# jinilover/floydWarshall

Measured on AMD Instinct MI355X. Metric: edge-relaxations/sec (N^3/t), N=16384 fp32, higher is better.
Workload: dtype f32

## Files before the change

floydwarshall_amd/_lib.py:

```python
import ctypes
import os

os.environ.setdefault("HSA_ENABLE_IPC_MODE_LEGACY", "0")

PKG = os.path.dirname(os.path.abspath(__file__))
LIB_PATH = os.environ.get("FWX_LIB_PATH") or os.path.join(PKG, "libfwx.so")

FWX_OK = 0
FWX_ERR_INVALID = -1
FWX_ERR_NO_DEVICE = -2
FWX_ERR_HIP = -3
FWX_ERR_OOM = -4
FWX_ERR_CYCLE = -5
FWX_ERR_CAPACITY = -6
FWX_ERR_UNSUPPORTED = -7
FWX_ERR_RCCL = -8
FWX_ERR_INTERNAL = -9

FWX_ABI_VERSION = 3
FWX_F32, FWX_F64 = 0, 1
FWX_ENGINE_AUTO, FWX_ENGINE_PERK, FWX_ENGINE_FUSED = 0, 1, 2
FWX_UPDATE_SHARDS = 256
FWX_FUSED_BLOCK = 64
FWX_BATCH_MAX_N = 128
# ... 42 lines not shown

class FwxMultiTiming(ctypes.Structure):
    _fields_ = [("struct_size", ctypes.c_uint32), ("steps", c_i32), ("pivots_per_step", c_i32),
                ("partitions", c_i32), ("bulk_us", ctypes.c_float), ("bulk_mean_us", ctypes.c_float),
                ("lookahead_us", ctypes.c_float), ("panel_us", ctypes.c_float),
                ("exchange_us", ctypes.c_float), ("chain_us", ctypes.c_float),
                ("chain_over_bulk", ctypes.c_float)]


class FwxError(RuntimeError):
    def __init__(self, status, what):
        self.status = status
        msg = lib().fwx_strerror(status).decode()
        extra = ""
        if status == FWX_ERR_HIP:
            extra = " (hipError_t %d)" % lib().fwx_last_hip_error()
        super().__init__("%s: %s%s" % (what, msg, extra))


SIGNATURES = {
    "fwx_abi_version": (ctypes.c_int, []),
    "fwx_device_count": (ctypes.c_int, []),
    "fwx_strerror": (ctypes.c_char_p, [ctypes.c_int]),
    "fwx_last_hip_error": (ctypes.c_int, []),
    "fwx_hip_versions": (ctypes.c_int, [ctypes.POINTER(c_i32), ctypes.POINTER(c_i32)]),
    "fwx_test_fail_after": (ctypes.c_int, [c_i32]),
    "fwx_test_kernel_forms": (ctypes.c_int, [ctypes.POINTER(ctypes.c_uint64), ctypes.c_int]),
    "fwx_test_kernel_form_name": (ctypes.c_char_p, [ctypes.c_int]),
    "fwx_test_perk_pivots": (ctypes.c_int, [ctypes.POINTER(ctypes.c_uint64), ctypes.c_int]),
    "fwx_test_perk_fold": (ctypes.c_int, []),
    "fwx_test_perk_walk": (ctypes.c_int, []),
    "fwx_test_perk_deep": (ctypes.c_int, [ctypes.POINTER(ctypes.c_uint64), ctypes.c_int]),
    "fwx_test_perk_tile": (ctypes.c_int, [ctypes.POINTER(ctypes.c_uint64), ctypes.c_int]),
    "fwx_test_perk_wide": (ctypes.c_int, [ctypes.POINTER(ctypes.c_uint64), ctypes.c_int]),
    "fwx_solve_f64": (ctypes.c_int, [c_i32, c_vp, c_vp, c_vp, ctypes.POINTER(FwxOpts)]),
    "fwx_solve_f32": (ctypes.c_int, [c_i32, c_vp, c_vp, c_vp, ctypes.POINTER(FwxOpts)]),
    "fwx_follow_path": (ctypes.c_int, [c_i32, c_vp, c_i32, c_i32, c_vp, c_i32]),
    "fwx_matrix_create": (ctypes.c_int, [ctypes.POINTER(c_vp), c_i32, c_i32, c_i32, c_i32, c_i32]),
    "fwx_matrix_upload": (ctypes.c_int, [c_vp, c_vp, c_vp, c_vp]),
    "fwx_matrix_solve": (ctypes.c_int, [c_vp, ctypes.POINTER(FwxOpts)]),
    "fwx_matrix_download": (ctypes.c_int, [c_vp, c_vp, c_vp, c_vp]),
    "fwx_matrix_query": (ctypes.c_int, [c_vp, c_i32, c_i32, ctypes.POINTER(ctypes.c_double), c_vp,
                                        c_i32]),
    "fwx_matrix_destroy": (ctypes.c_int, [c_vp]),
    "fwx_matrix_keep_input": (ctypes.c_int, [c_vp]),
    "fwx_matrix_patch_input": (ctypes.c_int, [c_vp, c_i32, c_vp, c_vp, c_vp, c_vp]),
    "fwx_matrix_enable_resume": (ctypes.c_int, [c_vp, c_i32]),
    "fwx_matrix_resume_bytes": (ctypes.c_int, [c_vp, c_i32, ctypes.POINTER(ctypes.c_uint64)]),
    "fwx_device_memory": (ctypes.c_int, [c_i32, ctypes.POINTER(ctypes.c_uint64),
                                         ctypes.POINTER(ctypes.c_uint64)]),
    "fwx_matrix_resolve": (ctypes.c_int, [c_vp, c_i32, c_vp, c_vp, c_vp, c_vp, ctypes.POINTER(FwxOpts),
                                          ctypes.POINTER(c_i32)]),
    "fwx_matrix_enable_path_log": (ctypes.c_int, [c_vp]),
    "fwx_matrix_path_log_count": (ctypes.c_int, [c_vp, ctypes.POINTER(ctypes.c_uint64)]),
    "fwx_matrix_query_exact": (ctypes.c_int, [c_vp, c_i32, c_i32, ctypes.POINTER(ctypes.c_double),
                                              c_vp, c_i32]),
    "fwx_matrix_query_exact_batch": (ctypes.c_int, [c_vp, c_i32, c_vp, c_vp, c_vp, c_vp, c_i32]),
    "fwx_matrix_create_multi": (ctypes.c_int, [ctypes.POINTER(c_vp), c_i32, c_i32, c_i32, c_i32, c_i32,
                                               ctypes.POINTER(c_i32), c_i32]),
    "fwx_matrix_create_part": (ctypes.c_int, [ctypes.POINTER(c_vp), c_i32, c_i32, c_i32, c_i32, c_i32, c_i32, c_i32,
                                              c_vp, c_vp]),
    "fwx_matrix_part_rows": (ctypes.c_int, [c_vp, c_i32, ctypes.POINTER(c_i32), ctypes.POINTER(c_i32)]),
    "fwx_matrix_domain_bits": (ctypes.c_int, [c_vp, ctypes.POINTER(c_i32)]),
    "fwx_matrix_set_domain": (ctypes.c_int, [c_vp, c_i32]),
    "fwx_matrix_parts": (ctypes.c_int, [c_vp, ctypes.POINTER(c_i32)]),
    "fwx_matrix_set_timing": (ctypes.c_int, [c_vp, c_i32]),
# ... 106 lines not shown
```

floydwarshall_amd/csrc/fwx_api.hip:

```cpp
#include <hip/hip_runtime.h>
#include <stddef.h>
#include <stdint.h>
#include <stdlib.h>
#include <string.h>

#include <cmath>
#include <new>

#include "fwx.h"
#include "fwx_guard.h"
#include "fwx_handle.h"
#include "fwx_internal.h"
#include "fwx_kernels.h"
#include "fwx_query.h"

using namespace fwxi;

namespace {

template <typename T>
int fused_block(const fwx_slab *sl, int k0, int bt, const T *w, const int32_t *wh,
                const fwx_fused_scratch *sc, const fwx_trace *tr, unsigned long long *d_updates,
                bool nonneg, hipStream_t s, int skip_lo = 0, int skip_hi = 0)
{
// ... 821 lines not shown
    return fwx::KF_COUNT;
}

int fwx_test_perk_pivots(uint64_t *launches, int reset)
{
    for (int i = 0; i < 5; ++i) {
        const uint64_t v = reset ? g_perk_launches[i].exchange(0, std::memory_order_relaxed)
                                 : g_perk_launches[i].load(std::memory_order_relaxed);
        if (launches) launches[i] = v;
    }
    return perk_pivots();
}

int fwx_test_perk_fold(void) { return perk_fold_compare() ? 1 : 0; }

int fwx_test_perk_walk(void) { return perk_walk() ? 1 : 0; }

int fwx_test_perk_deep(uint64_t *deep_launches, int reset)
{
    const uint64_t v = reset ? g_perk_deep_launches.exchange(0, std::memory_order_relaxed)
                             : g_perk_deep_launches.load(std::memory_order_relaxed);
    if (deep_launches) *deep_launches = v;
    return perk_deep() ? 1 : 0;
}

int fwx_test_perk_tile(uint64_t *launches, int reset)
{
    const uint64_t v = reset ? g_perk_tile_launches.exchange(0, std::memory_order_relaxed)
                             : g_perk_tile_launches.load(std::memory_order_relaxed);
    if (launches) *launches = v;
    return perk_tile_min_n();
}

int fwx_test_perk_wide(uint64_t *wide_launches, int reset)
{
    const uint64_t v = reset ? g_perk_wide_launches.exchange(0, std::memory_order_relaxed)
                             : g_perk_wide_launches.load(std::memory_order_relaxed);
    if (wide_launches) *wide_launches = v;
    return perk_wide() ? 1 : 0;
}

const char *fwx_test_kernel_form_name(int form)
{
    static const char *const names[] = {
#define FWX_KERNEL_FORM_NAME(name) #name,
        FWX_KERNEL_FORM_LIST(FWX_KERNEL_FORM_NAME)
#undef FWX_KERNEL_FORM_NAME
    };
    return form >= 0 && form < fwx::KF_COUNT ? names[form] : nullptr;
}

const char *fwx_strerror(int status)
{
    switch (status) {
    case FWX_OK: return "ok";
    case FWX_ERR_INVALID: return "invalid argument";
    case FWX_ERR_NO_DEVICE: return "no HIP device visible (libfwx has no CPU fallback)";
    case FWX_ERR_HIP: return "HIP runtime error";
    case FWX_ERR_OOM: return "out of memory";
    case FWX_ERR_CYCLE: return "next-hop walk does not reach the destination (cycle)";
    case FWX_ERR_CAPACITY: return "output buffer too small";
    case FWX_ERR_UNSUPPORTED: return "unsupported option combination";
    case FWX_ERR_RCCL: return "RCCL could not be loaded or an RCCL call failed";
    case FWX_ERR_INTERNAL: return "internal error (an exception was stopped at the C ABI)";
    default: return "unknown status";
    }
// ... 691 lines not shown
```

floydwarshall_amd/csrc/fwx_fused.hip:

```cpp
#include <hip/hip_runtime.h>
#include <type_traits>
#include <stdint.h>
#include <stdlib.h>

#include "fwx_kernels.h"

#pragma clang fp contract(off)

namespace fwx {

namespace {

template <typename T> __device__ __forceinline__ T qnan();
template <> __device__ __forceinline__ float qnan<float>() { return __builtin_nanf(""); }
template <> __device__ __forceinline__ double qnan<double>() { return __builtin_nan(""); }

__device__ __forceinline__ float fmax_t(float a, float b)
{
    float d;
    asm("v_max_f32 %0, %1, %2" : "=v"(d) : "v"(a), "v"(b));
    return d;
}
__device__ __forceinline__ double fmax_t(double a, double b)
{
// ... 946 lines not shown
        for (int q = 0; q < RI / 4; ++q) {
            const F32x4 cv = *reinterpret_cast<const F32x4 *>(&sCp[u][ti * RI + q * 4]);
#pragma unroll
            for (int e = 0; e < 4; ++e) c[q * 4 + e] = cv[e];
        }
#pragma unroll
        for (int h = 0; h < NH; ++h) {
            const F32x4 wq = *reinterpret_cast<const F32x4 *>(&sWp[u][h * 64 + tj * 4]);
#pragma unroll
            for (int e = 0; e < 4; ++e) wv[h][e] = wq[e];
        }
#pragma unroll
        for (int r = 0; r < RI; ++r)
#pragma unroll
            for (int h = 0; h < NH; ++h)
#pragma unroll
                for (int e = 0; e < 4; ++e) {
                    float p;
                    asm("v_mul_f32 %0, %1, %2" : "=v"(p) : "v"(c[r]), "v"(wv[h][e]));
                    x[r][h][e] = x[r][h][e] < p ? p : x[r][h][e];
                }
    }
}

__device__ __forceinline__ int sign_bits(F32x4 v)
{
    typedef int I4 __attribute__((ext_vector_type(4)));
    const I4 b = __builtin_bit_cast(I4, v);
    return b[0] | b[1] | b[2] | b[3];
}

template <int MINW, int RI, int NH>
__global__ __launch_bounds__(256, MINW) void relax_tile(float *rate, int n, int k0, const float *w,
                                                        const float *ct, int ct_ld, int force_cmp)
{
    typedef float V4 __attribute__((ext_vector_type(4)));
    constexpr int TI = 16 * RI, TJ = 64 * NH, HJ = 64, BS = 16, HP = BS / 2, NS = B / BS;
    static_assert(TI == 128 && TJ == 128, "every thread stages both operands: 8 pivot pairs x 32 vectors");

    __shared__ __attribute__((aligned(16))) float sW[2][HP][2][TJ];
    __shared__ __attribute__((aligned(16))) float sC[2][HP][2][TI];
    __shared__ __attribute__((aligned(16))) int sVote[2][4];

    const int tid = threadIdx.x;
    const int i_base = blockIdx.y * TI;
    const int j_base = blockIdx.x * TJ;
    const int ti = tid >> 4, tj = tid & 15;
    const int i0 = i_base + ti * RI;
    const int sp = tid >> 5, sv = tid & 31;

    auto voted = [&](int buf) -> bool {
        typedef int I4 __attribute__((ext_vector_type(4)));
        const I4 v = *reinterpret_cast<const I4 *>(&sVote[buf][0]);
        return __builtin_amdgcn_readfirstlane(v[0] | v[1] | v[2] | v[3]) != 0;
    };
    auto x_bits = [&](const V4 (&x)[RI][NH]) -> int {
        unsigned m = 0;
#pragma unroll
        for (int r = 0; r < RI; ++r)
#pragma unroll
            for (int h = 0; h < NH; ++h)
#pragma unroll
                for (int e = 0; e < 4; ++e) {
                    const float f = x[r][h][e];
                    const unsigned b = __builtin_bit_cast(unsigned, f);
                    m = b > m ? b : m;
                }
        return m > 0x7f800000u ? (int)0x80000000u : 0;
    };
    const bool interior = i_base + TI <= n && j_base + TJ <= n &&
                          !(i_base < j_base + TJ && j_base < i_base + TI) &&
                          (k0 + B <= j_base || k0 >= j_base + TJ);

    const float nanv = qnan<float>();
    const int sj = j_base + sv * 4, si = i_base + sv * 4;
    const bool sj_ok = sj < n, si_ok = si < n;
    const float *wp = w + (size_t)(2 * sp) * n + (sj_ok ? sj : 0);
    const float *cp = ct + (size_t)(2 * sp) * ct_ld + (si_ok ? si : 0);
    int kcol = k0 + 2 * sp - sj;
    V4 pw[2], pc[2];
    auto prefetch = [&]() {
        pw[0] = *reinterpret_cast<const V4 *>(wp);
        pw[1] = *reinterpret_cast<const V4 *>(wp + n);
        pc[0] = *reinterpret_cast<const V4 *>(cp);
        pc[1] = *reinterpret_cast<const V4 *>(cp + ct_ld);
        wp += (size_t)BS * n;
        cp += (size_t)BS * ct_ld;
    };
    auto commit = [&](int buf, int extra) {
        int bits = extra;
#pragma unroll
        for (int u = 0; u < 2; ++u) {
            V4 a = pw[u], c = pc[u];
#pragma unroll
            for (int e = 0; e < 4; ++e) {
                a[e] = (!sj_ok || kcol + u == e) ? nanv : a[e];
                c[e] = si_ok ? c[e] : nanv;
            }
            *reinterpret_cast<V4 *>(&sW[buf][sp][u][sv * 4]) = a;
            *reinterpret_cast<V4 *>(&sC[buf][sp][u][sv * 4]) = c;
            bits |= sign_bits(a) | sign_bits(c);
        }
        kcol += BS;
        sVote[buf][tid >> 6] = __builtin_amdgcn_ballot_w64(bits < 0) != 0 ? 1 : 0;
    };

    prefetch();
    V4 x[RI][NH];
    if (interior) {
        const float *xp = rate + (size_t)i0 * n + j_base + tj * 4;
#pragma unroll
        for (int r = 0; r < RI; ++r)
#pragma unroll
            for (int h = 0; h < NH; ++h) x[r][h] = *reinterpret_cast<const V4 *>(xp + (size_t)r * n + h * HJ);
    } else {
#pragma unroll
        for (int r = 0; r < RI; ++r) {
            const int i = min(i0 + r, n - 1);
#pragma unroll
            for (int h = 0; h < NH; ++h) {
                const int j = j_base + h * HJ + tj * 4;
                x[r][h] = *reinterpret_cast<const V4 *>(rate + (size_t)i * n + (j < n ? j : n - 4));
            }
        }
    }
    __builtin_amdgcn_s_waitcnt(FWX_WAIT_VMCNT0);
    commit(0, x_bits(x));
    __syncthreads();

    bool cmp = force_cmp != 0;
    int buf = 0;
#pragma unroll 1
    for (int s = 0; s < NS; ++s, buf ^= 1) {
        const bool more = s + 1 < NS;
        cmp |= voted(buf);
        if (more) prefetch();
        const int nmax = cmp ? 0 : HP;
#pragma unroll 1
        for (int tp = 0; tp < nmax; ++tp) max_fold_pair<RI, NH>(sW[buf][tp], sC[buf][tp], ti, tj, x);
#pragma unroll 1
        for (int tp = nmax; tp < HP; ++tp) cmp_fold_pair<RI, NH>(sW[buf][tp], sC[buf][tp], ti, tj, x);
        if (more) {
            commit(buf ^ 1, 0);
            __syncthreads();
        }
    }

    if (interior) {
        float *xp = rate + (size_t)i0 * n + j_base + tj * 4;
#pragma unroll
        for (int r = 0; r < RI; ++r)
#pragma unroll
            for (int h = 0; h < NH; ++h) *reinterpret_cast<V4 *>(xp + (size_t)r * n + h * HJ) = x[r][h];
        return;
    }
    if (i_base < j_base + TJ && j_base < i_base + TI) {
#pragma unroll
        for (int r = 0; r < RI; ++r) {
            const int i = i0 + r;
            if (i >= n) continue;
#pragma unroll
            for (int h = 0; h < NH; ++h) {
                const int j = j_base + h * HJ + tj * 4;
                if (i >= j && i < j + 4) x[r][h][i - j] = rate[(size_t)i * n + i];
            }
        }
        __builtin_amdgcn_s_waitcnt(FWX_WAIT_VMCNT0);
// ... 1276 lines not shown
            return hipGetLastError();
        }
        if (tight && a.next && !a.hops) {
            note_form(a.plog.last ? KF_PANELS_NEXT_TRACE_F32 : KF_PANELS_NEXT_F32);
            if (a.plog.last)
                hipLaunchKernelGGL(fused_panels_next_f32<true>, grid, block, 0, s, row_wgs, a.rate, a.next, a.n, a.k0,
                                   a.bt, w_out, a.ct, a.cnt, a.ct_ld, a.plog.last, a.plog.at_row, a.plog.at_col);
            else
                hipLaunchKernelGGL(fused_panels_next_f32<false>, grid, block, 0, s, row_wgs, a.rate, a.next, a.n, a.k0,
                                   a.bt, w_out, a.ct, a.cnt, a.ct_ld, nullptr, nullptr, nullptr);
            return hipGetLastError();
        }
    }
    const bool max_form = !a.plog.last && !a.next && a.nonneg;
    note_form(sizeof(T) == 4 ? (max_form ? KF_PANELS_MAX_F32 : KF_PANELS_F32)
                             : (max_form ? KF_PANELS_MAX_F64 : KF_PANELS_F64));
    if (a.plog.last) {
        if (a.hops) FWX_PANELS(true, true, true); else FWX_PANELS(true, true, false);
    } else if (a.next) {
        if (a.hops) FWX_PANELS(true, false, true); else FWX_PANELS(true, false, false);
    } else if (a.nonneg) {
        hipLaunchKernelGGL((fused_panels<T, false, false, false, true>), grid, block, 0, s, row_wgs, a.rate,
                           a.next, a.n, a.k0, a.bt, w_out, a.ct, a.cnt, a.ct_ld, a.plog.last, a.plog.at_row,
                           a.plog.at_col, a.hops, wh_out, a.cht);
    } else {
        FWX_PANELS(false, false, false);
    }
#undef FWX_PANELS
    return hipGetLastError();
}
template hipError_t launch_fused_panels<float>(const FusedArgs<float> &, float *, int32_t *, hipStream_t);
template hipError_t launch_fused_panels<double>(const FusedArgs<double> &, double *, int32_t *, hipStream_t);

hipError_t launch_relax_tile(const RelaxKtArgs<float> &a, hipStream_t s)
{
    if (a.n <= 0) return hipSuccess;
    if (a.np != B || a.n < B || a.n % 4 || a.ct_ld % 4 || a.ct_ld < a.n || (uintptr_t)a.rate % 16 || (uintptr_t)a.w % 16 ||
        (uintptr_t)a.ct % 16 || a.k < 0 || a.k + a.np > a.n || a.updates)
        return hipErrorInvalidValue;
    const unsigned tiles = (unsigned)((a.n + 127) / 128);
    note_form(KF_RELAX_K);
    hipLaunchKernelGGL((relax_tile<3, 8, 2>), dim3(tiles, tiles), dim3(256), 0, s, a.rate, a.n, a.k, a.w, a.ct,
                       a.ct_ld, a.fold_compare ? 1 : 0);
    return hipGetLastError();
}

template hipError_t launch_fused_relax<float>(const FusedArgs<float> &, hipStream_t, int, int);
template hipError_t launch_fused_relax<double>(const FusedArgs<double> &, hipStream_t, int, int);
template hipError_t launch_fused_colpanel<float>(const FusedArgs<float> &, hipStream_t);
template hipError_t launch_fused_colpanel<double>(const FusedArgs<double> &, hipStream_t);
template hipError_t launch_fused_main<float>(const FusedArgs<float> &, int, int, hipStream_t, int,
                                             int, FusedCols);
template hipError_t launch_fused_main<double>(const FusedArgs<double> &, int, int, hipStream_t, int,
                                              int, FusedCols);
template hipError_t launch_fused_panel<float>(const float *, int, int, int, float *, hipStream_t, PathLog,
                                              const int32_t *, int32_t *);
template hipError_t launch_fused_panel<double>(const double *, int, int, int, double *, hipStream_t,
                                               PathLog, const int32_t *, int32_t *);

}

#ifdef FWX_CLOCK_PROBE
extern "C" __attribute__((visibility("default"))) int fwx_debug_clock(unsigned long long *out, int reset)
{
    if (out && hipMemcpyFromSymbol(out, HIP_SYMBOL(fwx::g_clk), 24) != hipSuccess) return -1;
    if (reset) {
        const unsigned long long z[3] = {0, 0, 0};
        if (hipMemcpyToSymbol(HIP_SYMBOL(fwx::g_clk), z, 24) != hipSuccess) return -1;
    }
    return 0;
}
#endif
```

floydwarshall_amd/csrc/fwx_internal.h:

```cpp
#ifndef FWX_INTERNAL_H
#define FWX_INTERNAL_H

#include <hip/hip_runtime.h>
#include <algorithm>
#include <mutex>
#include <new>
#include <type_traits>
#include <vector>
#include <limits.h>
#include <stddef.h>
#include <stdlib.h>
#include <stdint.h>
#include <string.h>

#include "fwx.h"
#include "fwx_kernels.h"

static_assert(FWX_UPDATE_SHARDS == FWX_UPDATE_SHARDS_K, "shard count mismatch");

namespace fwxi {

inline thread_local int g_last_hip = 0;

#define FWX_HIP(call)                                                                              \
// ... 383 lines not shown

#define FWX_PERK_PIVOTS_DEFAULT 8
inline int perk_pivots()
{
    if (const char *e = getenv("FWX_PERK_PIVOTS")) {
        char *end = nullptr;
        const long v = strtol(e, &end, 10);
        if (end != e && *end == '\0' && (v == 1 || v == 2 || v == 4 || v == 8)) return (int)v;
    }
    return FWX_PERK_PIVOTS_DEFAULT;
}

inline bool perk_wide()
{
    const char *e = getenv("FWX_PERK_WIDE");
    return !(e && !strcmp(e, "0"));
}

inline bool perk_walk()
{
    const char *e = getenv("FWX_PERK_WALK");
    return !(e && !strcmp(e, "0"));
}

inline bool perk_deep()
{
    const char *e = getenv("FWX_PERK_DEEP");
    return !(e && !strcmp(e, "0"));
}

#define FWX_PERK_TILE_MIN_N_DEFAULT 1024
inline int perk_tile_min_n() { return (int)env_digits("FWX_PERK_TILE_MIN_N", 0, INT_MAX, FWX_PERK_TILE_MIN_N_DEFAULT); }

inline bool perk_fold_compare()
{
    const char *e = getenv("FWX_PERK_FOLD");
    return e && !strcmp(e, "compare");
}

#define FWX_BATCH_WAVE_MAX_N_DEFAULT FWX_BATCH_WAVE_N
inline int batch_wave_max_n()
{
    return (int)env_digits("FWX_BATCH_WAVE_MAX_N", 0, FWX_BATCH_WAVE_N, FWX_BATCH_WAVE_MAX_N_DEFAULT);
}

#define FWX_BATCH_MID_MIN_N_DEFAULT (FWX_BATCH_MAX_N + 1)
inline int batch_mid_min_n()
{
    return (int)env_digits("FWX_BATCH_MID_MIN_N", 1, FWX_BATCH_MID_MIN_N_DEFAULT, FWX_BATCH_MID_MIN_N_DEFAULT);
}

#define FWX_BATCH_LARGE_MIN_N_DEFAULT (FWX_BATCH_MID_MAX_N + 1)
inline int batch_large_min_n()
{
    return (int)env_digits("FWX_BATCH_LARGE_MIN_N", 1, FWX_BATCH_LARGE_MIN_N_DEFAULT, FWX_BATCH_LARGE_MIN_N_DEFAULT);
}

#define FWX_BATCH_LISTS_BUDGET_BYTES ((long long)64 << 20)
inline long long batch_lists_chunk(int n, int cap)
{
    const long long per_item = 4ll * ((long long)cap + 3ll * ((long long)n + 2) + 4);
    long long fit = FWX_BATCH_LISTS_BUDGET_BYTES / per_item;
    if (fit < 1) fit = 1;
    return env_digits("FWX_BATCH_LISTS_CHUNK", 1, fit - 1, fit);
}

inline std::atomic<uint64_t> g_perk_launches[5];
inline std::atomic<uint64_t> g_perk_wide_launches;
inline std::atomic<uint64_t> g_perk_deep_launches;
inline std::atomic<uint64_t> g_perk_tile_launches;

template <typename T> inline size_t perk_kt_ws_bytes(int n)
{
    const size_t ld = ((size_t)n + 3) & ~(size_t)3;
    return (size_t)FWX_FUSED_B * ((size_t)n + ld) * sizeof(T);
}
class PerkScratch {
public:
    static int get(hipStream_t s, size_t bytes, void **out)
    {
        int dev = 0, cur = 0;
        FWX_HIP(hipGetDevice(&cur));
        dev = cur;
        if (s) FWX_HIP(hipStreamGetDevice(s, &dev));
        Pool &p = pool();
        std::lock_guard<std::mutex> lk(p.mu);
        Entry *e = nullptr;
        for (Entry &x : p.all)
            if (x.s == s && x.dev == dev) { e = &x; break; }
        if (!e) {
            if (p.all.size() >= kMax) {
                size_t lru = 0;
                for (size_t i = 1; i < p.all.size(); ++i)
                    if (p.all[i].used < p.all[lru].used) lru = i;
                if (p.all[lru].p) (void)hipFree(p.all[lru].p);
                p.all.erase(p.all.begin() + (long)lru);
            }
            p.all.push_back(Entry{dev, s, nullptr, 0, 0});
            e = &p.all.back();
        }
        e->used = ++p.clock;
        if (e->cap < bytes) {
            if (e->p) {
                if (s) (void)hipStreamSynchronize(s);
                (void)hipFree(e->p);
                e->p = nullptr; e->cap = 0;
            }
            if (dev != cur) FWX_HIP(hipSetDevice(dev));
            const hipError_t err = hipMalloc(&e->p, bytes);
            if (dev != cur) (void)hipSetDevice(cur);
            FWX_HIP(err);
            e->cap = bytes;
        }
        *out = e->p;
        return FWX_OK;
    }

private:
    static constexpr size_t kMax = 16;
    struct Entry { int dev; hipStream_t s; void *p; size_t cap; uint64_t used; };
    struct Pool { std::mutex mu; std::vector<Entry> all; uint64_t clock = 0; };
    static Pool &pool() { static Pool *p = new Pool(); return *p; }
};

template <typename T>
inline int relax_range_kt(T *rate, int n, int k_begin, int k_end, int serpentine, int np,
                          unsigned long long *d_updates, hipStream_t s, void *ws)
{
    const size_t ld = ((size_t)n + 3) & ~(size_t)3;
    if (!ws) {
        const int rc0 = PerkScratch::get(s, perk_kt_ws_bytes<T>(n), &ws);
        if (rc0) return rc0;
    }
    T *const w = (T *)ws, *const ct = w + (size_t)FWX_FUSED_B * n;

    fwx::FusedArgs<T> pa;
    pa.rate = rate; pa.next = nullptr; pa.rows = n; pa.n = n; pa.row0 = 0; pa.w = nullptr; pa.ct = ct;
    pa.cnt = nullptr; pa.ct_ld = (int)ld; pa.updates = nullptr; pa.nonneg = false;
    fwx::RelaxKtArgs<T> a;
    a.rate = rate; a.ct_ld = (int)ld; a.n = n; a.updates = d_updates;
    a.temporal_bytes = perk_temporal_bytes((size_t)n * n * sizeof(T));
    a.store_bytes = perk_store_bytes();
    a.fold_compare = perk_fold_compare();
    a.walk = perk_walk();
    fwx::RelaxArgs<T> a1;
    a1.rate = rate; a1.next = nullptr; a1.hops = nullptr; a1.phops = nullptr; a1.rows = n; a1.n = n; a1.row0 = 0;
    a1.updates = d_updates; a1.temporal_bytes = a.temporal_bytes; a1.store_bytes = a.store_bytes;
    const int rev = FWX_XCD_SERPENTINE && a.temporal_bytes >= 0 ? 2 : 1;
    Throttle thr;
    int sweeps = 0;
    auto after = [&](hipError_t e, int slot, int groups = 1) -> int {
        if (e == hipErrorInvalidValue) return FWX_ERR_INVALID;
        FWX_HIP(e);
        g_perk_launches[slot].fetch_add((uint64_t)groups, std::memory_order_relaxed);
        if (groups >= 2) g_perk_wide_launches.fetch_add((uint64_t)groups / 2, std::memory_order_relaxed);
        if (groups >= 4) g_perk_deep_launches.fetch_add((uint64_t)groups / 4, std::memory_order_relaxed);
        if (groups == 8) g_perk_tile_launches.fetch_add(1, std::memory_order_relaxed);
        return thr.tick(s);
    };
    const bool wide = np == 8 && !d_updates && std::is_same<T, float>::value && perk_wide();
    const int g_top = wide ? (a.walk && perk_deep() ? 32 : 16) : np;
    const int tile_min_n = perk_tile_min_n();
    const bool tile = g_top == 32 && tile_min_n > 0 && n >= tile_min_n && n >= FWX_FUSED_B;
    for (int k0 = k_begin; k0 < k_end; k0 += FWX_FUSED_B) {
        const int bt = std::min(FWX_FUSED_B, k_end - k0);
        int t = 0;
        if (bt >= 2) {
            pa.k0 = k0; pa.bt = bt;
            if (const int rc = after(fwx::launch_fused_panels<T>(pa, w, nullptr, s), 4)) return rc;
            if constexpr (std::is_same<T, float>::value) {
                if (tile && bt == FWX_FUSED_B) {
                    a.k = k0; a.np = bt; a.w = w; a.ct = ct;
                    a.flip = 0;
                    if (const int rc = after(fwx::launch_relax_tile(a, s), 3, 8)) return rc;
                    t = bt;
                }
            }
            for (int g = g_top; g >= 2; g >>= 1)
                for (; bt - t >= g; t += g) {
                    a.k = k0 + t; a.np = g; a.w = w + (size_t)t * n; a.ct = ct + (size_t)t * ld;
                    a.flip = serpentine ? rev * (sweeps++ & 1) : 0;
                    if (const int rc = after(fwx::launch_relax_kt<T>(a, s), g >= 8 ? 3 : g == 4 ? 2 : 1, g >= 16 ? g / 8 : 1))
                        return rc;
                }
        }
        for (; t < bt; ++t) {
            a1.k = k0 + t; a1.prow = rate + (size_t)a1.k * n;
            a1.flip = serpentine ? rev * (sweeps++ & 1) : 0;
            if (const int rc = after(fwx::launch_relax<T>(a1, s), 0)) return rc;
        }
    }
    return FWX_OK;
}

template <typename T>
inline int relax_range(T *rate, int32_t *next, int32_t *hops, int rows, int n, int row0, const T *prow0,
                const int32_t *phops0, int64_t stride, int k_begin, int k_end, int serpentine,
                unsigned long long *d_updates, hipStream_t s, fwx::PathLog plog = fwx::PathLog(),
                int skip_lo = 0, int skip_hi = 0, const int32_t *pnext0 = nullptr, void *kt_ws = nullptr)
{
    const int np = perk_pivots();
    if (np > 1 && !next && !hops && !plog.last && row0 == 0 && rows == n && skip_hi <= skip_lo &&
        n % (16 / (int)sizeof(T)) == 0 && (uintptr_t)rate % 16 == 0 && stride == n &&
        prow0 == rate + (size_t)k_begin * n && k_end - k_begin >= 2)
        return relax_range_kt<T>(rate, n, k_begin, k_end, serpentine, np, d_updates, s, kt_ws);
    fwx::RelaxArgs<T> a;
    Throttle thr;
    a.rate = rate; a.next = next; a.hops = hops;
    a.rows = rows; a.n = n; a.row0 = row0; a.updates = d_updates; a.plog = plog;
    a.skip_lo = skip_lo; a.skip_hi = skip_hi;
    a.temporal_bytes = perk_temporal_bytes((size_t)rows * n * sizeof(T));
    a.store_bytes = perk_store_bytes();
    const int rev = FWX_XCD_SERPENTINE && a.temporal_bytes >= 0 ? 2 : 1;
    for (int k = k_begin; k < k_end; ++k) {
        a.prow = prow0 + (int64_t)(k - k_begin) * stride;
        a.phops = phops0 ? phops0 + (int64_t)(k - k_begin) * stride : nullptr;
        a.pnext = pnext0 ? pnext0 + (int64_t)(k - k_begin) * stride : nullptr;
        a.k = k;
        a.flip = serpentine ? rev * (k & 1) : 0;
        const hipError_t e = fwx::launch_relax<T>(a, s);
        if (e == hipErrorInvalidValue) return FWX_ERR_INVALID;
        FWX_HIP(e);
        const int rc = thr.tick(s);
        if (rc) return rc;
    }
// ... 27 lines not shown
```

floydwarshall_amd/csrc/fwx_kernels.h:

```cpp
#ifndef FWX_KERNELS_H
#define FWX_KERNELS_H

#include <hip/hip_runtime.h>
#include <stdint.h>

#include <atomic>

#define FWX_UPDATE_SHARDS_K 256

namespace fwx {

struct PathLog {
    int32_t *last = nullptr;
    int32_t *at_col = nullptr;
    int32_t *at_row = nullptr;
};

#define FWX_KERNEL_FORM_LIST(X)                                                                    \
    X(SMALL_SOLVE)                                              \
    X(RELAX_K)                                                      \
    X(ROWPANEL_F32)                                                        \
    X(ROWPANEL_F64)                                                                                \
    X(COLPANEL_F32)                                                     \
    X(COLPANEL_F64)                                                                                \
// ... 46 lines not shown
    int flip;
    long long temporal_bytes = -1;
    int store_bytes = 0;
    int skip_lo = 0, skip_hi = 0;
    unsigned long long *updates;
    PathLog plog;
};

template <typename T> hipError_t launch_relax(const RelaxArgs<T> &a, hipStream_t s);

#define FWX_PERK_KT_RPB 8
#define FWX_PERK_KT_UNROLL 8
#define FWX_PERK_KT16_RPB 16
#define FWX_PERK_KT16_UNROLL 8
#define FWX_PERK_WALK_RPB 16
#define FWX_PERK_WALK_UNROLL 8
#define FWX_PERK_WALK_POL 0
#define FWX_PERK_WALK_ROLL false
#define FWX_PERK_DEEP_RPB 64
#define FWX_PERK_DEEP_UNROLL 8
template <typename T> struct RelaxKtArgs {
    T *rate;
    const T *w;
    const T *ct;
    int ct_ld, n, k, np;
    int flip;
    long long temporal_bytes = -1;
    int store_bytes = 0;
    bool fold_compare = false;
    bool walk = false;
    unsigned long long *updates = nullptr;
};
template <typename T> hipError_t launch_relax_kt(const RelaxKtArgs<T> &a, hipStream_t s);
hipError_t launch_relax_tile(const RelaxKtArgs<float> &a, hipStream_t s);

#define FWX_SMALL_N 128
template <typename T>
hipError_t launch_small_solve(T *rate, int32_t *next, int32_t *hops, int n, int k_begin, int k_end,
                              unsigned long long *updates, PathLog plog, hipStream_t s);

#define FWX_BATCH_WAVE_N 16
template <typename T>
hipError_t launch_batch_solve(T *rate, int32_t *next, int32_t *hops, int count, int n, long long stride,
                              int k_begin, int k_end, unsigned long long *updates_each, int wave_max_n,
                              hipStream_t s, PathLog plog = PathLog());

#define FWX_MID_N 256
#ifndef FWX_MID_B
#define FWX_MID_B 16
#endif
template <typename T>
hipError_t launch_batch_mid(T *rate, int32_t *next, int32_t *hops, int count, int n, long long stride, int k_begin,
                            int k_end, unsigned long long *updates_each, hipStream_t s, PathLog plog = PathLog());

#define FWX_LARGE_N 1024
#define FWX_LARGE_B 16
#define FWX_LARGE_S 48
#ifndef FWX_LARGE_TR
#define FWX_LARGE_TR 16
#endif
#ifndef FWX_LARGE_ROWS
#define FWX_LARGE_ROWS 4
#endif
#ifndef FWX_LARGE_TC
#define FWX_LARGE_TC 256
#endif
#define FWX_LARGE_SCRATCH_BYTES(n) ((size_t)(n) * (2 * FWX_LARGE_B * 16))
// ... 69 lines not shown
```

include/fwx.h:

```cpp
#ifndef FWX_H
#define FWX_H

#include <stddef.h>
#include <stdint.h>

#ifdef __cplusplus
extern "C" {
#endif

#define FWX_ABI_VERSION 3

typedef enum fwx_status {
    FWX_OK = 0,
    FWX_ERR_INVALID = -1,
    FWX_ERR_NO_DEVICE = -2,
    FWX_ERR_HIP = -3,
    FWX_ERR_OOM = -4,
    FWX_ERR_CYCLE = -5,
    FWX_ERR_CAPACITY = -6,
    FWX_ERR_UNSUPPORTED = -7,
    FWX_ERR_RCCL = -8,
    FWX_ERR_INTERNAL = -9
} fwx_status;

// ... 3 lines not shown
    FWX_ENGINE_AUTO = 0,
    FWX_ENGINE_PERK = 1,
    FWX_ENGINE_FUSED = 2
} fwx_engine;

typedef struct fwx_opts {
    uint32_t struct_size;
    int32_t device;
    int32_t engine;
    int32_t k_begin;
    int32_t k_end;
    int32_t block;
    int32_t serpentine;
    uint64_t *updates_out;
    void *stream;
    int32_t use_stream;
    int32_t reserved0;
} fwx_opts;

int fwx_abi_version(void);
int fwx_device_count(void);
const char *fwx_strerror(int status);
int fwx_last_hip_error(void);
int fwx_hip_versions(int32_t *built_against, int32_t *runtime);
int fwx_test_fail_after(int32_t countdown);
int fwx_test_kernel_forms(uint64_t *seen, int reset);
const char *fwx_test_kernel_form_name(int form);
int fwx_test_perk_pivots(uint64_t *launches, int reset);
int fwx_test_perk_wide(uint64_t *wide_launches, int reset);
int fwx_test_perk_fold(void);
int fwx_test_perk_walk(void);
int fwx_test_perk_deep(uint64_t *deep_launches, int reset);
int fwx_test_perk_tile(uint64_t *launches, int reset);

int fwx_solve_f64(int32_t n, double *rate, int32_t *next, int32_t *hops, const fwx_opts *opts);
int fwx_solve_f32(int32_t n, float *rate, int32_t *next, int32_t *hops, const fwx_opts *opts);

#define FWX_BATCH_MAX_N 128
int fwx_solve_batch_f64(int32_t count, int32_t n, double *rate, int32_t *next, int32_t *hops,
                        uint64_t *updates_each, const fwx_opts *opts);
int fwx_solve_batch_f32(int32_t count, int32_t n, float *rate, int32_t *next, int32_t *hops,
                        uint64_t *updates_each, const fwx_opts *opts);
int fwx_dev_solve_batch(int32_t count, int32_t n, int32_t dtype, void *rate, int32_t *next, int32_t *hops,
                        int64_t stride, int32_t k_begin, int32_t k_end,
                        unsigned long long *d_updates_each, void *stream);
int fwx_test_batch_wave_max_n(void);

#define FWX_BATCH_MID_MAX_N 256
int fwx_solve_batch_mid_f64(int32_t count, int32_t n, double *rate, int32_t *next, int32_t *hops,
                            uint64_t *updates_each, const fwx_opts *opts);
int fwx_solve_batch_mid_f32(int32_t count, int32_t n, float *rate, int32_t *next, int32_t *hops,
                            uint64_t *updates_each, const fwx_opts *opts);
int fwx_dev_solve_batch_mid(int32_t count, int32_t n, int32_t dtype, void *rate, int32_t *next, int32_t *hops,
                            int64_t stride, int32_t k_begin, int32_t k_end,
                            unsigned long long *d_updates_each, void *stream);
int fwx_test_batch_mid_min_n(void);
int fwx_test_batch_mid_block(void);

#define FWX_BATCH_LARGE_MAX_N 1024
#define FWX_BATCH_LARGE_SCRATCH_BYTES(n) ((size_t)(n) * 512)
int fwx_solve_batch_large_f64(int32_t count, int32_t n, double *rate, int32_t *next, int32_t *hops,
                              uint64_t *updates_each, const fwx_opts *opts);
int fwx_solve_batch_large_f32(int32_t count, int32_t n, float *rate, int32_t *next, int32_t *hops,
                              uint64_t *updates_each, const fwx_opts *opts);
int fwx_dev_solve_batch_large(int32_t count, int32_t n, int32_t dtype, void *rate, int32_t *next, int32_t *hops,
                              int64_t stride, int32_t k_begin, int32_t k_end,
// ... 229 lines not shown
```

Baseline: 28220 billion.

## Pair pivot blocks in tile relax and overlap next panels on side stream

```diff
diff --git a/floydwarshall_amd/_lib.py b/floydwarshall_amd/_lib.py
--- a/floydwarshall_amd/_lib.py
+++ b/floydwarshall_amd/_lib.py
@@ -98,6 +98,7 @@
     "fwx_test_perk_walk": (ctypes.c_int, []),
     "fwx_test_perk_deep": (ctypes.c_int, [ctypes.POINTER(ctypes.c_uint64), ctypes.c_int]),
     "fwx_test_perk_tile": (ctypes.c_int, [ctypes.POINTER(ctypes.c_uint64), ctypes.c_int]),
+    "fwx_test_perk_pair": (ctypes.c_int, [ctypes.POINTER(ctypes.c_uint64), ctypes.c_int]),
     "fwx_test_perk_wide": (ctypes.c_int, [ctypes.POINTER(ctypes.c_uint64), ctypes.c_int]),
     "fwx_solve_f64": (ctypes.c_int, [c_i32, c_vp, c_vp, c_vp, ctypes.POINTER(FwxOpts)]),
     "fwx_solve_f32": (ctypes.c_int, [c_i32, c_vp, c_vp, c_vp, ctypes.POINTER(FwxOpts)]),
diff --git a/floydwarshall_amd/csrc/fwx_api.hip b/floydwarshall_amd/csrc/fwx_api.hip
--- a/floydwarshall_amd/csrc/fwx_api.hip
+++ b/floydwarshall_amd/csrc/fwx_api.hip
@@ -877,6 +877,14 @@
     return perk_tile_min_n();
 }
 
+int fwx_test_perk_pair(uint64_t *launches, int reset)
+{
+    const uint64_t v = reset ? g_perk_pair_launches.exchange(0, std::memory_order_relaxed)
+                             : g_perk_pair_launches.load(std::memory_order_relaxed);
+    if (launches) *launches = v;
+    return perk_pair_min_n();
+}
+
 int fwx_test_perk_wide(uint64_t *wide_launches, int reset)
 {
     const uint64_t v = reset ? g_perk_wide_launches.exchange(0, std::memory_order_relaxed)
diff --git a/floydwarshall_amd/csrc/fwx_fused.hip b/floydwarshall_amd/csrc/fwx_fused.hip
--- a/floydwarshall_amd/csrc/fwx_fused.hip
+++ b/floydwarshall_amd/csrc/fwx_fused.hip
@@ -1002,19 +1002,35 @@
 
 template <int MINW, int RI, int NH>
 __global__ __launch_bounds__(256, MINW) void relax_tile(float *rate, int n, int k0, const float *w,
-                                                        const float *ct, int ct_ld, int force_cmp)
+                                                        const float *ct, int ct_ld, int force_cmp, int ns, int sel,
+                                                        int tx)
 {
     typedef float V4 __attribute__((ext_vector_type(4)));
-    constexpr int TI = 16 * RI, TJ = 64 * NH, HJ = 64, BS = 16, HP = BS / 2, NS = B / BS;
+    constexpr int TI = 16 * RI, TJ = 64 * NH, HJ = 64, BS = 16, HP = BS / 2;
     static_assert(TI == 128 && TJ == 128, "every thread stages both operands: 8 pivot pairs x 32 vectors");
 
     __shared__ __attribute__((aligned(16))) float sW[2][HP][2][TJ];
     __shared__ __attribute__((aligned(16))) float sC[2][HP][2][TI];
     __shared__ __attribute__((aligned(16))) int sVote[2][4];
 
+    int bx = blockIdx.x, by = blockIdx.y;
+    if (sel == TILES_EXCEPT) {
+        bx += bx >= tx ? 1 : 0;
+        by += by >= tx ? 1 : 0;
+    } else if (sel == TILES_CROSS) {
+        __builtin_amdgcn_s_setprio(2);
+        const int tiles = ((int)gridDim.x + 1) >> 1;
+        if (bx < tiles) {
+            by = tx;
+        } else {
+            by = bx - tiles;
+            by += by >= tx ? 1 : 0;
+            bx = tx;
+        }
+    }
     const int tid = threadIdx.x;
-    const int i_base = blockIdx.y * TI;
-    const int j_base = blockIdx.x * TJ;
+    const int i_base = by * TI;
+    const int j_base = bx * TJ;
     const int ti = tid >> 4, tj = tid & 15;
     const int i0 = i_base + ti * RI;
     const int sp = tid >> 5, sv = tid & 31;
@@ -1040,7 +1056,7 @@
     };
     const bool interior = i_base + TI <= n && j_base + TJ <= n &&
                           !(i_base < j_base + TJ && j_base < i_base + TI) &&
-                          (k0 + B <= j_base || k0 >= j_base + TJ);
+                          (k0 + ns * BS <= j_base || k0 >= j_base + TJ);
 
     const float nanv = qnan<float>();
     const int sj = j_base + sv * 4, si = i_base + sv * 4;
@@ -1101,8 +1117,8 @@
     bool cmp = force_cmp != 0;
     int buf = 0;
 #pragma unroll 1
-    for (int s = 0; s < NS; ++s, buf ^= 1) {
-        const bool more = s + 1 < NS;
+    for (int s = 0; s < ns; ++s, buf ^= 1) {
+        const bool more = s + 1 < ns;
         cmp |= voted(buf);
         if (more) prefetch();
         const int nmax = cmp ? 0 : HP;
@@ -2445,16 +2461,21 @@
 template hipError_t launch_fused_panels<float>(const FusedArgs<float> &, float *, int32_t *, hipStream_t);
 template hipError_t launch_fused_panels<double>(const FusedArgs<double> &, double *, int32_t *, hipStream_t);
 
-hipError_t launch_relax_tile(const RelaxKtArgs<float> &a, hipStream_t s)
+hipError_t launch_relax_tile(const RelaxKtArgs<float> &a, hipStream_t s, TileSel sel, int tx)
 {
     if (a.n <= 0) return hipSuccess;
-    if (a.np != B || a.n < B || a.n % 4 || a.ct_ld % 4 || a.ct_ld < a.n || (uintptr_t)a.rate % 16 || (uintptr_t)a.w % 16 ||
-        (uintptr_t)a.ct % 16 || a.k < 0 || a.k + a.np > a.n || a.updates)
+    if ((a.np != B && a.np != 2 * B) || a.n < B || a.n % 4 || a.ct_ld % 4 || a.ct_ld < a.n || (uintptr_t)a.rate % 16 ||
+        (uintptr_t)a.w % 16 || (uintptr_t)a.ct % 16 || a.k < 0 || a.k + a.np > a.n || a.updates)
         return hipErrorInvalidValue;
-    const unsigned tiles = (unsigned)((a.n + 127) / 128);
+    const int tiles = (a.n + 127) / 128;
+    if (sel != TILES_ALL && (tx < 0 || tx >= tiles)) return hipErrorInvalidValue;
+    const dim3 grid = sel == TILES_ALL      ? dim3((unsigned)tiles, (unsigned)tiles)
+                      : sel == TILES_EXCEPT ? dim3((unsigned)(tiles - 1), (unsigned)(tiles - 1))
+                                            : dim3((unsigned)(2 * tiles - 1));
+    if (grid.x == 0) return hipSuccess;
     note_form(KF_RELAX_K);
-    hipLaunchKernelGGL((relax_tile<3, 8, 2>), dim3(tiles, tiles), dim3(256), 0, s, a.rate, a.n, a.k, a.w, a.ct,
-                       a.ct_ld, a.fold_compare ? 1 : 0);
+    hipLaunchKernelGGL((relax_tile<3, 8, 2>), grid, dim3(256), 0, s, a.rate, a.n, a.k, a.w, a.ct, a.ct_ld,
+                       a.fold_compare ? 1 : 0, a.np / 16, (int)sel, tx);
     return hipGetLastError();
 }
 
diff --git a/floydwarshall_amd/csrc/fwx_internal.h b/floydwarshall_amd/csrc/fwx_internal.h
--- a/floydwarshall_amd/csrc/fwx_internal.h
+++ b/floydwarshall_amd/csrc/fwx_internal.h
@@ -439,6 +439,9 @@
 #define FWX_PERK_TILE_MIN_N_DEFAULT 1024
 inline int perk_tile_min_n() { return (int)env_digits("FWX_PERK_TILE_MIN_N", 0, INT_MAX, FWX_PERK_TILE_MIN_N_DEFAULT); }
 
+#define FWX_PERK_PAIR_MIN_N_DEFAULT 5120
+inline int perk_pair_min_n() { return (int)env_digits("FWX_PERK_PAIR_MIN_N", 0, INT_MAX, FWX_PERK_PAIR_MIN_N_DEFAULT); }
+
 inline bool perk_fold_compare()
 {
     const char *e = getenv("FWX_PERK_FOLD");
@@ -476,15 +479,20 @@
 inline std::atomic<uint64_t> g_perk_wide_launches;
 inline std::atomic<uint64_t> g_perk_deep_launches;
 inline std::atomic<uint64_t> g_perk_tile_launches;
+inline std::atomic<uint64_t> g_perk_pair_launches;
 
 template <typename T> inline size_t perk_kt_ws_bytes(int n)
 {
     const size_t ld = ((size_t)n + 3) & ~(size_t)3;
     return (size_t)FWX_FUSED_B * ((size_t)n + ld) * sizeof(T);
 }
+struct PerkSide {
+    hipStream_t s = nullptr;
+    hipEvent_t main_done = nullptr, chain_done = nullptr;
+};
 class PerkScratch {
 public:
-    static int get(hipStream_t s, size_t bytes, void **out)
+    static int get(hipStream_t s, size_t bytes, void **out, PerkSide *side = nullptr)
     {
         int dev = 0, cur = 0;
         FWX_HIP(hipGetDevice(&cur));
@@ -501,9 +509,10 @@
                 for (size_t i = 1; i < p.all.size(); ++i)
                     if (p.all[i].used < p.all[lru].used) lru = i;
                 if (p.all[lru].p) (void)hipFree(p.all[lru].p);
+                release(p.all[lru].side);
                 p.all.erase(p.all.begin() + (long)lru);
             }
-            p.all.push_back(Entry{dev, s, nullptr, 0, 0});
+            p.all.push_back(Entry{dev, s, nullptr, 0, 0, PerkSide()});
             e = &p.all.back();
         }
         e->used = ++p.clock;
@@ -519,13 +528,30 @@
             FWX_HIP(err);
             e->cap = bytes;
         }
+        if (side && !e->side.chain_done) {
+            if (dev != cur) FWX_HIP(hipSetDevice(dev));
+            hipError_t err = hipStreamCreateWithFlags(&e->side.s, hipStreamNonBlocking);
+            if (err == hipSuccess) err = hipEventCreateWithFlags(&e->side.main_done, hipEventDisableTiming);
+            if (err == hipSuccess) err = hipEventCreateWithFlags(&e->side.chain_done, hipEventDisableTiming);
+            if (err != hipSuccess) release(e->side);
+            if (dev != cur) (void)hipSetDevice(cur);
+            FWX_HIP(err);
+        }
+        if (side) *side = e->side;
         *out = e->p;
         return FWX_OK;
     }
 
 private:
     static constexpr size_t kMax = 16;
-    struct Entry { int dev; hipStream_t s; void *p; size_t cap; uint64_t used; };
+    struct Entry { int dev; hipStream_t s; void *p; size_t cap; uint64_t used; PerkSide side; };
+    static void release(PerkSide &d)
+    {
+        if (d.main_done) (void)hipEventDestroy(d.main_done);
+        if (d.chain_done) (void)hipEventDestroy(d.chain_done);
+        if (d.s) (void)hipStreamDestroy(d.s);
+        d = PerkSide();
+    }
     struct Pool { std::mutex mu; std::vector<Entry> all; uint64_t clock = 0; };
     static Pool &pool() { static Pool *p = new Pool(); return *p; }
 };
@@ -534,12 +560,36 @@
 inline int relax_range_kt(T *rate, int n, int k_begin, int k_end, int serpentine, int np,
                           unsigned long long *d_updates, hipStream_t s, void *ws)
 {
+    constexpr int Bq = FWX_FUSED_B;
     const size_t ld = ((size_t)n + 3) & ~(size_t)3;
+    const bool wide = np == 8 && !d_updates && std::is_same<T, float>::value && perk_wide();
+    const int g_top = wide ? (perk_walk() && perk_deep() ? 32 : 16) : np;
+    const int tile_min_n = perk_tile_min_n();
+    const bool tile = g_top == 32 && tile_min_n > 0 && n >= tile_min_n && n >= Bq;
+    const int k_a = (k_begin + 2 * Bq - 1) / (2 * Bq) * (2 * Bq);
+    const int pair_min_n = perk_pair_min_n();
+    bool pair = tile && !ws && pair_min_n > 0 && n >= pair_min_n && k_begin % Bq == 0 && k_end - k_a >= 4 * Bq;
+    if (pair) {
+        hipStreamCaptureStatus cap = hipStreamCaptureStatusNone;
+        if (hipStreamIsCapturing(s, &cap) != hipSuccess) {
+            (void)hipGetLastError();
+            pair = false;
+        } else if (cap != hipStreamCaptureStatusNone) {
+            pair = false;
+        }
+    }
+    const int sets = pair ? 4 : 1;
+    PerkSide side;
     if (!ws) {
-        const int rc0 = PerkScratch::get(s, perk_kt_ws_bytes<T>(n), &ws);
+        const int rc0 = PerkScratch::get(s, (size_t)sets * perk_kt_ws_bytes<T>(n), &ws, pair ? &side : nullptr);
         if (rc0) return rc0;
     }
-    T *const w = (T *)ws, *const ct = w + (size_t)FWX_FUSED_B * n;
+    T *const w_all = (T *)ws, *const ct_all = w_all + (size_t)sets * Bq * n;
+    T *w = w_all, *ct = ct_all;
+    auto use_set = [&](int q) {
+        w = w_all + (size_t)(q & (sets - 1)) * Bq * n;
+        ct = ct_all + (size_t)(q & (sets - 1)) * Bq * ld;
+    };
 
     fwx::FusedArgs<T> pa;
     pa.rate = rate; pa.next = nullptr; pa.rows = n; pa.n = n; pa.row0 = 0; pa.w = nullptr; pa.ct = ct;
@@ -559,29 +609,36 @@
     auto after = [&](hipError_t e, int slot, int groups = 1) -> int {
         if (e == hipErrorInvalidValue) return FWX_ERR_INVALID;
         FWX_HIP(e);
-        g_perk_launches[slot].fetch_add((uint64_t)groups, std::memory_order_relaxed);
-        if (groups >= 2) g_perk_wide_launches.fetch_add((uint64_t)groups / 2, std::memory_order_relaxed);
-        if (groups >= 4) g_perk_deep_launches.fetch_add((uint64_t)groups / 4, std::memory_order_relaxed);
-        if (groups == 8) g_perk_tile_launches.fetch_add(1, std::memory_order_relaxed);
+        if (slot >= 0) {
+            g_perk_launches[slot].fetch_add((uint64_t)groups, std::memory_order_relaxed);
+            if (groups >= 2) g_perk_wide_launches.fetch_add((uint64_t)groups / 2, std::memory_order_relaxed);
+            if (groups >= 4) g_perk_deep_launches.fetch_add((uint64_t)groups / 4, std::memory_order_relaxed);
+            if (groups >= 8) g_perk_tile_launches.fetch_add((uint64_t)groups / 8, std::memory_order_relaxed);
+            if (groups == 16) g_perk_pair_launches.fetch_add(1, std::memory_order_relaxed);
+        }
         return thr.tick(s);
     };
-    const bool wide = np == 8 && !d_updates && std::is_same<T, float>::value && perk_wide();
-    const int g_top = wide ? (a.walk && perk_deep() ? 32 : 16) : np;
-    const int tile_min_n = perk_tile_min_n();
-    const bool tile = g_top == 32 && tile_min_n > 0 && n >= tile_min_n && n >= FWX_FUSED_B;
-    for (int k0 = k_begin; k0 < k_end; k0 += FWX_FUSED_B) {
-        const int bt = std::min(FWX_FUSED_B, k_end - k0);
+    auto panels = [&](int k0, int bt, hipStream_t st) -> int {
+        pa.k0 = k0; pa.bt = bt; pa.ct = ct; pa.side = st != s;
+        return after(fwx::launch_fused_panels<T>(pa, w, nullptr, st), 4);
+    };
+    auto tiles = [&](int k0, int bt, hipStream_t st, fwx::TileSel sel, int tx) -> int {
+        if constexpr (std::is_same<T, float>::value) {
+            a.k = k0; a.np = bt; a.w = w; a.ct = ct;
+            a.flip = 0;
+            return after(fwx::launch_relax_tile(a, st, sel, tx), sel == fwx::TILES_CROSS ? -1 : 3, bt / 8);
+        } else {
+            return FWX_ERR_INVALID;
+        }
+    };
+    auto block = [&](int k0, int bt, bool panels_ready) -> int {
         int t = 0;
         if (bt >= 2) {
-            pa.k0 = k0; pa.bt = bt;
-            if (const int rc = after(fwx::launch_fused_panels<T>(pa, w, nullptr, s), 4)) return rc;
-            if constexpr (std::is_same<T, float>::value) {
-                if (tile && bt == FWX_FUSED_B) {
-                    a.k = k0; a.np = bt; a.w = w; a.ct = ct;
-                    a.flip = 0;
-                    if (const int rc = after(fwx::launch_relax_tile(a, s), 3, 8)) return rc;
-                    t = bt;
-                }
+            if (!panels_ready)
+                if (const int rc = panels(k0, bt, s)) return rc;
+            if (tile && bt == Bq) {
+                if (const int rc = tiles(k0, bt, s, fwx::TILES_ALL, 0)) return rc;
+                t = bt;
             }
             for (int g = g_top; g >= 2; g >>= 1)
                 for (; bt - t >= g; t += g) {
@@ -596,8 +653,67 @@
             a1.flip = serpentine ? rev * (sweeps++ & 1) : 0;
             if (const int rc = after(fwx::launch_relax<T>(a1, s), 0)) return rc;
         }
-    }
-    return FWX_OK;
+        return FWX_OK;
+    };
+    if (!pair) {
+        for (int k0 = k_begin; k0 < k_end; k0 += Bq)
+            if (const int rc = block(k0, std::min(Bq, k_end - k0), false)) return rc;
+        return FWX_OK;
+    }
+
+    const int nfull = (k_end - k_a) / Bq, pairs = nfull / 2;
+    auto k_of = [&](int q) { return k_a + q * Bq; };
+    bool chain_open = false;
+    auto join = [&]() -> hipError_t {
+        chain_open = false;
+        hipError_t e = hipEventRecord(side.chain_done, side.s);
+        if (e == hipSuccess) e = hipStreamWaitEvent(s, side.chain_done, 0);
+        return e;
+    };
+    auto run = [&]() -> int {
+        if (k_begin < k_a) {
+            use_set(-1);
+            if (const int rc = block(k_begin, Bq, false)) return rc;
+        }
+        use_set(0);
+        if (const int rc = panels(k_of(0), Bq, s)) return rc;
+        if (const int rc = tiles(k_of(0), Bq, s, fwx::TILES_CROSS, k_a / (2 * Bq))) return rc;
+        use_set(1);
+        if (const int rc = panels(k_of(1), Bq, s)) return rc;
+        for (int P = 0; P < pairs; ++P) {
+            const int q = 2 * P, ahead = std::min(2, nfull - (q + 2));
+            const int xn = k_of(q + 2) / (2 * Bq);
+            if (ahead > 0) {
+                FWX_HIP(hipEventRecord(side.main_done, s));
+                FWX_HIP(hipStreamWaitEvent(side.s, side.main_done, 0));
+                chain_open = true;
+                use_set(q);
+                if (const int rc = tiles(k_of(q), 2 * Bq, side.s, fwx::TILES_CROSS, xn)) return rc;
+                use_set(q + 2);
+                if (const int rc = panels(k_of(q + 2), Bq, side.s)) return rc;
+                if (ahead == 2) {
+                    if (const int rc = tiles(k_of(q + 2), Bq, side.s, fwx::TILES_CROSS, xn)) return rc;
+                    use_set(q + 3);
+                    if (const int rc = panels(k_of(q + 3), Bq, side.s)) return rc;
+                }
+            }
+            use_set(q);
+            if (const int rc = tiles(k_of(q), 2 * Bq, s, ahead > 0 ? fwx::TILES_EXCEPT : fwx::TILES_ALL, xn)) return rc;
+            if (chain_open) FWX_HIP(join());
+        }
+        if (nfull & 1) {
+            use_set(nfull - 1);
+            if (const int rc = block(k_of(nfull - 1), Bq, true)) return rc;
+        }
+        if (k_of(nfull) < k_end) {
+            use_set(nfull);
+            if (const int rc = block(k_of(nfull), k_end - k_of(nfull), false)) return rc;
+        }
+        return FWX_OK;
+    };
+    const int rc = run();
+    if (chain_open) (void)join();
+    return rc;
 }
 
 template <typename T>
diff --git a/floydwarshall_amd/csrc/fwx_kernels.h b/floydwarshall_amd/csrc/fwx_kernels.h
--- a/floydwarshall_amd/csrc/fwx_kernels.h
+++ b/floydwarshall_amd/csrc/fwx_kernels.h
@@ -102,7 +102,8 @@
     unsigned long long *updates = nullptr;
 };
 template <typename T> hipError_t launch_relax_kt(const RelaxKtArgs<T> &a, hipStream_t s);
-hipError_t launch_relax_tile(const RelaxKtArgs<float> &a, hipStream_t s);
+enum TileSel { TILES_ALL = 0, TILES_EXCEPT = 1, TILES_CROSS = 2 };
+hipError_t launch_relax_tile(const RelaxKtArgs<float> &a, hipStream_t s, TileSel sel = TILES_ALL, int tx = 0);
 
 #define FWX_SMALL_N 128
 template <typename T>
diff --git a/include/fwx.h b/include/fwx.h
--- a/include/fwx.h
+++ b/include/fwx.h
@@ -59,6 +59,7 @@
 int fwx_test_perk_walk(void);
 int fwx_test_perk_deep(uint64_t *deep_launches, int reset);
 int fwx_test_perk_tile(uint64_t *launches, int reset);
+int fwx_test_perk_pair(uint64_t *launches, int reset);
 
 int fwx_solve_f64(int32_t n, double *rate, int32_t *next, int32_t *hops, const fwx_opts *opts);
 int fwx_solve_f32(int32_t n, float *rate, int32_t *next, int32_t *hops, const fwx_opts *opts);
```

Measured after the change: 31340 billion (median of 6 runs). 1.11x the previous value.
